# huttered40/capital

Measured on AMD Instinct MI355X. Metric: TFLOP/s (whole node) Cholesky n=65536, algorithmic n^3/3, recursive cholinv factor(), inputs resident in HBM, higher is better.
Workload: dtype f64

## Files before the change

### capital_amd/csrc/gemm_f64.hip

```cpp
#include "capi_internal.h"
#include "gemm_plan.h"
#include <type_traits>

extern "C" int capi_internal_copy2d(capi_handle_t h, int64_t m, int64_t n, const double* A, int64_t lda, double* B, int64_t ldb);

typedef double d4_t __attribute__((ext_vector_type(4)));
typedef double d2_t __attribute__((ext_vector_type(2)));

namespace {

constexpr int NTHREADS = 256;
using gemm_plan::BK, gemm_plan::SK;
template <int TS> struct tile_cfg {
  static constexpr int TILE_LDS = TS * SK;
  static constexpr int STAGE_LDS = 2 * TILE_LDS;
  static constexpr int NQ = TS / 32;
  static constexpr int SUB = TS / 32;
};
constexpr int GROUP_M = 8;
template <int TS> __device__ __forceinline__ int rc_r(int tid, int q) { return 16 * ((tid >> 6) * (TS / 64) + (q >> 1)) + 2 * (tid & 7); }
__device__ __forceinline__ int rc_k(int tid, int q) { return 8 * (q & 1) + ((tid >> 3) & 7); }

struct GemmArgs {
  const double* A;
  const double* B;
  double* C;
  int64_t lda, ldb, ldc;
  int M, N, K;
  double alpha, beta;
  int out_uplo;
  int tri_side;
  int tri_eff_upper;
  int tri_unit;
  int a_vec, b_vec;
  int splitk, k_per_split;
  int k_rotate;
  double* slab;
  int64_t slab_ld, slab_stride;
  int tiles_m, tiles_n, ntiles;
  int batch;
  int64_t sa, sb, sc;
  int tail_base, tail_tm, tail_tn;
  int ts;
  int no_skip;
  int share_ab;
  int tri_dense;
  int tri_koff;
  int tri_block;
  int pid_base;
  int order;
  int a_tiled, c_tiled;
  unsigned long long* stamp;
};

__device__ __forceinline__ void stamp_begin(const GemmArgs& p) {
  if (p.stamp && threadIdx.x == 0) atomicMin(p.stamp, (unsigned long long)wall_clock64());
}
__device__ __forceinline__ void stamp_end(const GemmArgs& p) {
  if (p.stamp && threadIdx.x == 0) atomicMin(p.stamp + 1, ~(unsigned long long)wall_clock64());
}

template <int TS, bool KC>
__device__ __forceinline__ void panel_load(const double* __restrict__ X, int64_t ld, int r0, int R, int k0, int kend,
                                           int tid, bool vec_ok, d2_t (&v)[TS / 32]) {
  constexpr int NQ = TS / 32;
  if (KC) {
    const int kp = tid & 7, rb = tid >> 3;
    const int k = k0 + 2 * kp;
#pragma unroll
    for (int q = 0; q < NQ; ++q) {
      const int r = r0 + rb + 32 * q;
      d2_t val = {0.0, 0.0};
      if (r < R) {
        const double* p = X + (int64_t)r * ld + k;
        if (vec_ok && k + 1 < kend) {
          val = *(const d2_t*)p;
        } else {
          if (k < kend) val.x = p[0];
          if (k + 1 < kend) val.y = p[1];
        }
      }
      v[q] = val;
    }
  } else {
#pragma unroll
    for (int q = 0; q < NQ; ++q) {
      const int r = r0 + rc_r<TS>(tid, q);
      const int k = k0 + rc_k(tid, q);
      d2_t val = {0.0, 0.0};
      if (k < kend) {
        const double* p = X + (int64_t)k * ld + r;
        if (vec_ok && r + 1 < R) {
          val = *(const d2_t*)p;
        } else {
          if (r < R) val.x = p[0];
          if (r + 1 < R) val.y = p[1];
        }
      }
      v[q] = val;
    }
  }
}

template <int TS>
__device__ __forceinline__ void panel_load_fast(const double* __restrict__ base, int64_t s1, int64_t s2, d2_t (&v)[TS / 32]) {
#pragma unroll
  for (int q = 0; q < TS / 32; ++q) v[q] = *(const d2_t*)(base + (q & 1) * s1 + (q >> 1) * s2);
}

template <int TS, bool KC>
__device__ __forceinline__ void panel_mask(int r0, int k0, int tid, bool keep_ge, bool unit, d2_t (&v)[TS / 32]) {
#pragma unroll
  for (int q = 0; q < TS / 32; ++q) {
    int r[2], k[2];
    if (KC) {
      r[0] = r[1] = r0 + (tid >> 3) + 32 * q;
      k[0] = k0 + 2 * (tid & 7);
      k[1] = k[0] + 1;
    } else {
      r[0] = r0 + rc_r<TS>(tid, q);
      r[1] = r[0] + 1;
      k[0] = k[1] = k0 + rc_k(tid, q);
    }
    double e0 = v[q].x, e1 = v[q].y;
    if (keep_ge ? (k[0] < r[0]) : (k[0] > r[0])) e0 = 0.0;
    if (keep_ge ? (k[1] < r[1]) : (k[1] > r[1])) e1 = 0.0;
    if (unit) {
      if (k[0] == r[0]) e0 = 1.0;
      if (k[1] == r[1]) e1 = 1.0;
    }
    v[q].x = e0;
    v[q].y = e1;
  }
}

template <int TS, bool KC>
__device__ __forceinline__ void panel_store(double* __restrict__ L, int tid, const d2_t (&v)[TS / 32]) {
  if (KC) {
    const int kp = tid & 7, rb = tid >> 3;
#pragma unroll
    for (int q = 0; q < TS / 32; ++q) *(d2_t*)&L[(rb + 32 * q) * SK + 2 * kp] = v[q];
  } else {
#pragma unroll
    for (int q = 0; q < TS / 32; ++q) {
      double* d = &L[rc_r<TS>(tid, q) * SK + rc_k(tid, q)];
      d[0] = v[q].x;
      d[SK] = v[q].y;
    }
  }
}

__device__ __forceinline__ d2_t frag_read(const double* __restrict__ L, int row, int u, int g) {
  return *(const d2_t*)&L[row * SK + 8 * u + 2 * g];
}

template <int SUB, int COMP, bool ALL>
__device__ __forceinline__ void mfma_step(d4_t (&acc)[SUB][SUB], const d2_t (&af)[SUB], const d2_t (&bf)[SUB], unsigned keep) {
  constexpr unsigned FULL = (1u << (SUB * SUB)) - 1u;
  if (ALL || keep == FULL) {
#pragma unroll
    for (int a = 0; a < SUB; ++a)
#pragma unroll
      for (int b = 0; b < SUB; ++b)
        acc[a][b] = __builtin_amdgcn_mfma_f64_16x16x4f64(COMP ? bf[b].y : bf[b].x, COMP ? af[a].y : af[a].x, acc[a][b], 0, 0, 0);
  } else {
#pragma unroll
    for (int a = 0; a < SUB; ++a)
#pragma unroll
      for (int b = 0; b < SUB; ++b)
        if (keep & (1u << (a * SUB + b)))
          acc[a][b] = __builtin_amdgcn_mfma_f64_16x16x4f64(COMP ? bf[b].y : bf[b].x, COMP ? af[a].y : af[a].x, acc[a][b], 0, 0, 0);
  }
}

__device__ __forceinline__ void tile_of_dims(int out_uplo, int nm, int nn, int t, int& ti, int& tj, int order = 0) {
  if (out_uplo >= 0 && (order & 1)) {
    int first = 0, gsz = GROUP_M;
    for (;; first += GROUP_M) {
      gsz = min(nn - first, GROUP_M);
      const int cnt = gsz * (gsz + 1) / 2 + gsz * (nn - first - gsz);
      if (t < cnt || first + GROUP_M >= nn) break;
      t -= cnt;
    }
    const int ntri = gsz * (gsz + 1) / 2;
    int lo, hi;
    if (t < ntri) {
      hi = 0;
      while ((hi + 1) * (hi + 2) / 2 <= t) ++hi;
      lo = first + t - hi * (hi + 1) / 2;
      hi += first;
    } else {
      t -= ntri;
      hi = first + gsz + t / gsz;
      lo = first + t % gsz;
    }
    if (out_uplo == CAPI_UPPER) { ti = lo; tj = hi; } else { ti = hi; tj = lo; }
  } else if (out_uplo < 0) {
    const int in_group = GROUP_M * nn;
    const int group = t / in_group;
    const int first_m = group * GROUP_M;
    const int gsz = min(nm - first_m, GROUP_M);
    const int loc = t - group * in_group;
    ti = first_m + loc % gsz;
    tj = loc / gsz;
  } else {
    int hi = (int)((sqrt(8.0 * (double)t + 1.0) - 1.0) * 0.5);
    while ((int64_t)hi * (hi + 1) / 2 > t) --hi;
    while ((int64_t)(hi + 1) * (hi + 2) / 2 <= t) ++hi;
    const int lo = t - (int)((int64_t)hi * (hi + 1) / 2);
    if (out_uplo == CAPI_UPPER) { ti = lo; tj = hi; } else { ti = hi; tj = lo; }
  }
}

__device__ __forceinline__ void tile_of(const GemmArgs& p, int t, int& ti, int& tj) {
  if (p.tail_base > 0) {
    int ti128, tj128;
    tile_of_dims(p.out_uplo, p.tail_tm, p.tail_tn, p.tail_base + (t >> 2), ti128, tj128, p.order);
    ti = 2 * ti128 + (t & 1);
    tj = 2 * tj128 + ((t >> 1) & 1);
  } else {
    tile_of_dims(p.out_uplo, p.tiles_m, p.tiles_n, t, ti, tj, p.order);
  }
}

__device__ __forceinline__ void trmm_tile_of(const GemmArgs& p, int r, int& ti, int& tj) {
  const bool left = p.tri_side == CAPI_LEFT;
  const int nfree = left ? p.tiles_n : p.tiles_m, ntri = left ? p.tiles_m : p.tiles_n;
  int b = r / nfree;
  const int a = r - b * nfree;
  const bool longest_last = left ? !p.tri_eff_upper : (p.tri_eff_upper != 0);
  if (longest_last) b = ntri - 1 - b;
  ti = left ? b : a;
  tj = left ? a : b;
}

template <int TS, bool AK, bool BKC>
__global__ __launch_bounds__(NTHREADS, TS == 128 ? 2 : 4) void dgemm_tile_kernel(const GemmArgs p) {
  constexpr int BM = TS, BN = TS, SUB = tile_cfg<TS>::SUB, NQ = tile_cfg<TS>::NQ;
  constexpr int NW = NQ * ((AK ? 1 : 2) + (BKC ? 1 : 2));
  constexpr int TILE_LDS = tile_cfg<TS>::TILE_LDS, STAGE_LDS = tile_cfg<TS>::STAGE_LDS;
  extern __shared__ __attribute__((aligned(16))) double lds[];
  const int tid = threadIdx.x;
  const int lane = tid & 63, wave = tid >> 6;
  const int r16 = lane & 15, g = lane >> 4;
  const int wm = wave & 1, wn = wave >> 1;
  stamp_begin(p);

  const int nblk = gridDim.x, bid = blockIdx.x;
  const int xcd = bid & 7, qq = nblk >> 3, rr = nblk & 7;
  const int pid = p.pid_base + (xcd < rr ? xcd * (qq + 1) : rr * (qq + 1) + (xcd - rr) * qq) + (bid >> 3);
  int z = pid / p.ntiles;
  int ti, tj;
  if (p.tri_side >= 0 && p.splitk == 1 && !p.tri_block) { z = 0; trmm_tile_of(p, bid, ti, tj); }
  else tile_of(p, pid - z * p.ntiles, ti, tj);
  if (p.tail_base > 0) {
    if (ti >= p.tiles_m || tj >= p.tiles_n) return;
    if (p.out_uplo == CAPI_UPPER && ti > tj) return;
    if (p.out_uplo == CAPI_LOWER && tj > ti) return;
  }
  const int i0 = ti * BM, j0 = tj * BN;

  int klo = 0, khi = p.K;
  if (p.tri_side == CAPI_LEFT) {
    if (p.tri_eff_upper) klo = i0; else khi = min(p.K, i0 + BM);
  } else if (p.tri_side == CAPI_RIGHT) {
    if (p.tri_eff_upper) khi = min(p.K, p.tri_koff + j0 + BN); else klo = j0;
  }
  constexpr int kstep = BK;
  if (p.splitk > 1) {
    klo = max(klo, z * p.k_per_split);
    khi = min(khi, (z + 1) * p.k_per_split);
  }
  const int ntk = khi > klo ? (khi - klo + kstep - 1) / kstep : 0;
  const bool maskA = p.tri_side == CAPI_LEFT && !p.tri_dense, maskB = p.tri_side == CAPI_RIGHT && !p.tri_dense;
  const bool shareB = AK == BKC && p.share_ab && ti == tj;
  const bool keep_ge = (p.tri_side == CAPI_LEFT) == (p.tri_eff_upper != 0);

  d4_t acc[SUB][SUB];
#pragma unroll
  for (int a = 0; a < SUB; ++a)
#pragma unroll
    for (int b = 0; b < SUB; ++b) acc[a][b] = (d4_t){0.0, 0.0, 0.0, 0.0};

  const bool interior = (i0 + BM <= p.M) && (j0 + BN <= p.N) && p.a_vec && p.b_vec;
  const double* fa = AK ? p.A + (int64_t)(i0 + (tid >> 3)) * p.lda + klo + 2 * (tid & 7)
                     : p.A + (int64_t)(klo + rc_k(tid, 0)) * p.lda + i0 + rc_r<TS>(tid, 0);
  const double* fb = BKC ? p.B + (int64_t)(j0 + (tid >> 3)) * p.ldb + klo + 2 * (tid & 7)
                     : p.B + (int64_t)(klo + rc_k(tid, 0)) * p.ldb + j0 + rc_r<TS>(tid, 0);
  const int64_t qsa = AK ? 32 * p.lda : 8 * p.lda;
  const int64_t qsa2 = AK ? 64 * p.lda : 16;
  const int64_t qsb = BKC ? 32 * p.ldb : 8 * p.ldb;
  const int64_t qsb2 = BKC ? 64 * p.ldb : 16;
  const int64_t ksa = AK ? kstep : (int64_t)kstep * p.lda, ksb = BKC ? kstep : (int64_t)kstep * p.ldb;

  unsigned out_keep = (1u << (SUB * SUB)) - 1u;
  if (p.out_uplo >= 0 && ti == tj && !p.no_skip) {
#pragma unroll
    for (int a = 0; a < SUB; ++a)
#pragma unroll
      for (int b = 0; b < SUB; ++b) {
        const int rlo = wm * (TS / 2) + 16 * a, clo = wn * (TS / 2) + 16 * b;
        const bool on = p.out_uplo == CAPI_UPPER ? (rlo <= clo + 15) : (rlo + 15 >= clo);
        if (!on) out_keep &= ~(1u << (a * SUB + b));
      }
  }

  const int rot = (p.k_rotate && p.splitk > 1 && ntk > 1) ? (int)((int64_t)z * ntk / p.splitk) : 0;
  const int kfirst = klo + rot * kstep;
  d2_t ra[NQ], rb[NQ];
  if (ntk > 0) {
    panel_load<TS, AK>(p.A, p.lda, i0, p.M, kfirst, khi, tid, p.a_vec, ra);
    if (!shareB) panel_load<TS, BKC>(p.B, p.ldb, j0, p.N, kfirst, khi, tid, p.b_vec, rb);
    if (maskA && klo < i0 + BM && klo + BK > i0) panel_mask<TS, AK>(i0, klo, tid, keep_ge, p.tri_unit, ra);
    if (maskB && klo < j0 + BN && klo + BK > j0) panel_mask<TS, BKC>(j0, klo, tid, keep_ge, p.tri_unit, rb);
    panel_store<TS, AK>(lds, tid, ra);
    if (!shareB) panel_store<TS, BKC>(lds + TILE_LDS, tid, rb);
  }
  __syncthreads();

  int par = 0;
  auto iterate = [&](const int t, const int tnext, auto fast_tag) {
    constexpr bool FAST = decltype(fast_tag)::value;
    const double* La = lds + par * STAGE_LDS;
    const double* Lb = shareB ? La : La + TILE_LDS;
    const int kn = klo + tnext * kstep;
    const bool more = FAST || (tnext >= 0);
    if (FAST) {
      fa += ksa;
      fb += ksb;
      __builtin_amdgcn_s_setprio(1);
      panel_load_fast<TS>(fa, qsa, qsa2, ra);
      panel_load_fast<TS>(fb, qsb, qsb2, rb);
    } else if (more) {
      panel_load<TS, AK>(p.A, p.lda, i0, p.M, kn, khi, tid, p.a_vec, ra);
      if (!shareB) panel_load<TS, BKC>(p.B, p.ldb, j0, p.N, kn, khi, tid, p.b_vec, rb);
    }
    unsigned keep = (1u << (SUB * SUB)) - 1u;
    if (!FAST) {
      keep = out_keep;
      const int kk = klo + t * kstep;
      const bool band = p.tri_side == CAPI_LEFT ? (kk < i0 + BM && kk + BK > i0) : (kk < j0 + BN && kk + BK > j0);
      if (p.tri_side >= 0 && band && !p.no_skip && !p.tri_dense) {
#pragma unroll
        for (int a = 0; a < SUB; ++a)
#pragma unroll
          for (int b = 0; b < SUB; ++b) {
            bool on;
            if (p.tri_side == CAPI_LEFT) {
              const int rlo = i0 + wm * (TS / 2) + 16 * a;
              on = p.tri_eff_upper ? (kk + BK - 1 >= rlo) : (kk <= rlo + 15);
            } else {
              const int clo = j0 + wn * (TS / 2) + 16 * b;
              on = p.tri_eff_upper ? (kk <= clo + 15) : (kk + BK - 1 >= clo);
            }
            if (!on) keep &= ~(1u << (a * SUB + b));
          }
      }
    }
#pragma unroll
    for (int u = 0; u < 2; ++u) {
      d2_t af[SUB], bf[SUB];
#pragma unroll
      for (int a = 0; a < SUB; ++a) af[a] = frag_read(La, wm * (TS / 2) + a * 16 + r16, u, g);
#pragma unroll
      for (int b = 0; b < SUB; ++b) bf[b] = frag_read(Lb, wn * (TS / 2) + b * 16 + r16, u, g);
      if (!FAST) __builtin_amdgcn_s_setprio(1);
      mfma_step<SUB, 0, FAST>(acc, af, bf, keep);
      mfma_step<SUB, 1, FAST>(acc, af, bf, keep);
      if (FAST && u == 1) {
        double* Na = lds + (par ^ 1) * STAGE_LDS;
        panel_store<TS, AK>(Na, tid, ra);
        panel_store<TS, BKC>(Na + TILE_LDS, tid, rb);
        __builtin_amdgcn_sched_group_barrier(0x100, 2 * SUB, 0);
#pragma unroll
        for (int i = 0; i < 2 * NQ; ++i) {
          __builtin_amdgcn_sched_group_barrier(0x008, (SUB * SUB) / (2 * NQ), 0);
          __builtin_amdgcn_sched_group_barrier(0x020, 1, 0);
        }
#pragma unroll
        for (int i = 0; i < 2 * SUB; ++i) {
          __builtin_amdgcn_sched_group_barrier(0x008, (SUB * SUB) / (2 * SUB), 0);
          __builtin_amdgcn_sched_group_barrier(0x100, 1, 0);
        }
#pragma unroll
        for (int i = 0; i < NW; ++i) {
          __builtin_amdgcn_sched_group_barrier(0x008, (2 * SUB * SUB) / NW > 0 ? (2 * SUB * SUB) / NW : 1, 0);
          __builtin_amdgcn_sched_group_barrier(0x200, 1, 0);
        }
      }
      if (!FAST || u == 1) __builtin_amdgcn_s_setprio(0);
    }
    if (more && !FAST) {
      if (maskA && kn < i0 + BM && kn + BK > i0) panel_mask<TS, AK>(i0, kn, tid, keep_ge, p.tri_unit, ra);
      if (maskB && kn < j0 + BN && kn + BK > j0) panel_mask<TS, BKC>(j0, kn, tid, keep_ge, p.tri_unit, rb);
      double* Na = lds + (par ^ 1) * STAGE_LDS;
      panel_store<TS, AK>(Na, tid, ra);
      if (!shareB) panel_store<TS, BKC>(Na + TILE_LDS, tid, rb);
    }
    par ^= 1;
    __syncthreads();
  };
  const int nfast = (interior && khi - klo >= BK) ? (khi - klo - BK) / kstep : 0;
  int tb0 = ntk, tb1 = ntk;
  if (p.tri_side >= 0 && !p.tri_dense) {
    const int d0 = p.tri_side == CAPI_LEFT ? i0 : j0;
    tb0 = d0 > klo ? (d0 - klo) / BK : 0;
    tb1 = d0 + TS > klo ? (d0 + TS - klo + BK - 1) / BK : 0;
  }
  const double* const fa0 = fa;
  const double* const fb0 = fb;
  for (int seg = 0; seg < 2; ++seg) {
    const int tb = seg == 0 ? rot : 0, te = seg == 0 ? ntk : rot;
    const int after = (seg == 0 && rot > 0) ? 0 : -1;
    fa = fa0 + (int64_t)tb * ksa;
    fb = fb0 + (int64_t)tb * ksb;
    const int lim = min(nfast, te - 1);
    int t = tb;
    while (t < te) {
      const int fe = t + 1 < tb0 ? min(tb0 - 1, lim) : (t >= tb1 ? lim : t);
      for (; t < fe; ++t) iterate(t, t + 1, std::true_type{});
      const int ge = (t < tb1 && tb1 < lim) ? tb1 : te;
      const int t_in = t;
      for (; t < ge; ++t) iterate(t, t + 1 < te ? t + 1 : after, std::false_type{});
      fa += (int64_t)(t - t_in) * ksa;
      fb += (int64_t)(t - t_in) * ksb;
    }
  }

  auto element_ok = [&](int i, int j) {
    bool ok = (i < p.M) && (j < p.N);
    if (p.out_uplo == CAPI_UPPER) ok = ok && (i <= j);
    if (p.out_uplo == CAPI_LOWER) ok = ok && (i >= j);
    return ok;
  };
  if (p.splitk > 1) {
#pragma unroll
    for (int a = 0; a < SUB; ++a) {
      const int i = i0 + wm * (TS / 2) + a * 16 + r16;
#pragma unroll
      for (int b = 0; b < SUB; ++b)
#pragma unroll
        for (int reg = 0; reg < 4; ++reg) {
          const int j = j0 + wn * (TS / 2) + b * 16 + g + 4 * reg;
          if (element_ok(i, j)) p.slab[(int64_t)z * p.slab_stride + i + (int64_t)j * p.slab_ld] = acc[a][b][reg];
        }
    }
  } else if (p.beta == 0.0) {
#pragma unroll
    for (int a = 0; a < SUB; ++a) {
      const int i = i0 + wm * (TS / 2) + a * 16 + r16;
#pragma unroll
      for (int b = 0; b < SUB; ++b)
#pragma unroll
        for (int reg = 0; reg < 4; ++reg) {
          const int j = j0 + wn * (TS / 2) + b * 16 + g + 4 * reg;
          if (element_ok(i, j)) p.C[i + (int64_t)j * p.ldc] = p.alpha * acc[a][b][reg];
        }
    }
  } else {
#pragma unroll
    for (int a = 0; a < SUB; ++a) {
      const int i = i0 + wm * (TS / 2) + a * 16 + r16;
      double old[SUB][4];
#pragma unroll
      for (int b = 0; b < SUB; ++b)
#pragma unroll
        for (int reg = 0; reg < 4; ++reg) {
          const int j = j0 + wn * (TS / 2) + b * 16 + g + 4 * reg;
          const bool ok = element_ok(i, j);
          old[b][reg] = *(ok ? p.C + i + (int64_t)j * p.ldc : p.C);
        }
#pragma unroll
      for (int b = 0; b < SUB; ++b)
#pragma unroll
        for (int reg = 0; reg < 4; ++reg) {
          const int j = j0 + wn * (TS / 2) + b * 16 + g + 4 * reg;
          if (element_ok(i, j)) p.C[i + (int64_t)j * p.ldc] = p.alpha * acc[a][b][reg] + p.beta * old[b][reg];
        }
    }
  }
  stamp_end(p);
}

template <bool AK, bool BKC>
__global__ __launch_bounds__(NTHREADS, 2) void dtrmm_pair_kernel(const GemmArgs p) {
  constexpr int TS = 128, BM = TS, BN = TS, SUB = tile_cfg<TS>::SUB, NQ = tile_cfg<TS>::NQ;
  constexpr int NW = NQ * ((AK ? 1 : 2) + (BKC ? 1 : 2));
  constexpr int TILE_LDS = tile_cfg<TS>::TILE_LDS, STAGE_LDS = tile_cfg<TS>::STAGE_LDS;
  constexpr int kstep = BK;
  extern __shared__ __attribute__((aligned(16))) double lds[];
  const int tid = threadIdx.x;
  const int lane = tid & 63, wave = tid >> 6;
  const int r16 = lane & 15, g = lane >> 4;
  const int wm = wave & 1, wn = wave >> 1;
  stamp_begin(p);

  const int nblk = gridDim.x, bid = blockIdx.x;
  const int xcd = bid & 7, qq = nblk >> 3, rr = nblk & 7;
  const int pid = p.pid_base + (xcd < rr ? xcd * (qq + 1) : rr * (qq + 1) + (xcd - rr) * qq) + (bid >> 3);
  const bool left = p.tri_side == CAPI_LEFT;
  const int ntri = left ? p.tiles_m : p.tiles_n, nfree = left ? p.tiles_n : p.tiles_m, npair = ntri >> 1;
  int pb, fr;
  if (left) tile_of_dims(-1, npair, nfree, pid, pb, fr); else tile_of_dims(-1, nfree, npair, pid, fr, pb);
  const bool anchor0 = left ? !p.tri_eff_upper : (p.tri_eff_upper != 0);
  const bool maskA = left, maskB = !left;
  const bool keep_ge = left == (p.tri_eff_upper != 0);
  const int64_t ksa = AK ? kstep : (int64_t)kstep * p.lda, ksb = BKC ? kstep : (int64_t)kstep * p.ldb;
  const int64_t qsa = AK ? 32 * p.lda : 8 * p.lda;
  const int64_t qsa2 = AK ? 64 * p.lda : 16;
  const int64_t qsb = BKC ? 32 * p.ldb : 8 * p.ldb;
  const int64_t qsb2 = BKC ? 64 * p.ldb : 16;

  for (int ph = 0; ph < 2; ++ph) {
    const bool asc = (ph == 0) == anchor0;
    const int bt = asc ? pb : ntri - 1 - pb;
    const int ti = left ? bt : fr, tj = left ? fr : bt;
    const int i0 = ti * BM, j0 = tj * BN, d0 = left ? i0 : j0;
    const int klo = anchor0 ? 0 : d0, khi = anchor0 ? d0 + TS : p.K;
    const int ntk = (khi - klo) / kstep;
    const int tb0 = (d0 - klo) / BK, tb1 = tb0 + TS / BK;

    d4_t acc[SUB][SUB];
#pragma unroll
    for (int a = 0; a < SUB; ++a)
#pragma unroll
      for (int c = 0; c < SUB; ++c) acc[a][c] = (d4_t){0.0, 0.0, 0.0, 0.0};

    const double* const fa0 = AK ? p.A + (int64_t)(i0 + (tid >> 3)) * p.lda + klo + 2 * (tid & 7)
                              : p.A + (int64_t)(klo + rc_k(tid, 0)) * p.lda + i0 + rc_r<TS>(tid, 0);
    const double* const fb0 = BKC ? p.B + (int64_t)(j0 + (tid >> 3)) * p.ldb + klo + 2 * (tid & 7)
                              : p.B + (int64_t)(klo + rc_k(tid, 0)) * p.ldb + j0 + rc_r<TS>(tid, 0);
    const double* fa = fa0;
    const double* fb = fb0;
    const int64_t sa = asc ? ksa : -ksa, sb = asc ? ksb : -ksb;
    const int dir = asc ? 1 : -1;
    int t = asc ? 0 : ntk - 1;

    d2_t ra[NQ], rb[NQ];
    {
      const int kf = klo + t * kstep;
      panel_load<TS, AK>(p.A, p.lda, i0, p.M, kf, khi, tid, 1, ra);
      panel_load<TS, BKC>(p.B, p.ldb, j0, p.N, kf, khi, tid, 1, rb);
      if (maskA && t >= tb0 && t < tb1) panel_mask<TS, AK>(i0, kf, tid, keep_ge, p.tri_unit, ra);
      if (maskB && t >= tb0 && t < tb1) panel_mask<TS, BKC>(j0, kf, tid, keep_ge, p.tri_unit, rb);
      panel_store<TS, AK>(lds, tid, ra);
      panel_store<TS, BKC>(lds + TILE_LDS, tid, rb);
    }
    __syncthreads();

    int par = 0;
    auto iterate = [&](const int tc, const int tnext, auto fast_tag) {
      constexpr bool FAST = decltype(fast_tag)::value;
      const double* La = lds + par * STAGE_LDS;
      const double* Lb = La + TILE_LDS;
      const int kn = klo + tnext * kstep;
      const bool more = FAST || (tnext >= 0);
      if (FAST) {
        fa += sa;
        fb += sb;
        __builtin_amdgcn_s_setprio(1);
        panel_load_fast<TS>(fa, qsa, qsa2, ra);
        panel_load_fast<TS>(fb, qsb, qsb2, rb);
      } else if (more) {
        panel_load<TS, AK>(p.A, p.lda, i0, p.M, kn, khi, tid, 1, ra);
        panel_load<TS, BKC>(p.B, p.ldb, j0, p.N, kn, khi, tid, 1, rb);
      }
      unsigned keep = (1u << (SUB * SUB)) - 1u;
      if (!FAST) {
        const int kk = klo + tc * kstep;
        if (tc >= tb0 && tc < tb1 && !p.no_skip) {
#pragma unroll
          for (int a = 0; a < SUB; ++a)
#pragma unroll
            for (int c = 0; c < SUB; ++c) {
              bool on;
              if (left) {
                const int rlo = i0 + wm * (TS / 2) + 16 * a;
                on = p.tri_eff_upper ? (kk + BK - 1 >= rlo) : (kk <= rlo + 15);
              } else {
                const int clo = j0 + wn * (TS / 2) + 16 * c;
                on = p.tri_eff_upper ? (kk <= clo + 15) : (kk + BK - 1 >= clo);
              }
              if (!on) keep &= ~(1u << (a * SUB + c));
            }
        }
      }
#pragma unroll
      for (int u = 0; u < 2; ++u) {
        d2_t af[SUB], bf[SUB];
#pragma unroll
        for (int a = 0; a < SUB; ++a) af[a] = frag_read(La, wm * (TS / 2) + a * 16 + r16, u, g);
#pragma unroll
        for (int c = 0; c < SUB; ++c) bf[c] = frag_read(Lb, wn * (TS / 2) + c * 16 + r16, u, g);
        if (!FAST) __builtin_amdgcn_s_setprio(1);
        mfma_step<SUB, 0, FAST>(acc, af, bf, keep);
        mfma_step<SUB, 1, FAST>(acc, af, bf, keep);
        if (FAST && u == 1) {
          double* Na = lds + (par ^ 1) * STAGE_LDS;
          panel_store<TS, AK>(Na, tid, ra);
          panel_store<TS, BKC>(Na + TILE_LDS, tid, rb);
          __builtin_amdgcn_sched_group_barrier(0x100, 2 * SUB, 0);
#pragma unroll
          for (int i = 0; i < 2 * NQ; ++i) {
            __builtin_amdgcn_sched_group_barrier(0x008, (SUB * SUB) / (2 * NQ), 0);
            __builtin_amdgcn_sched_group_barrier(0x020, 1, 0);
          }
#pragma unroll
          for (int i = 0; i < 2 * SUB; ++i) {
            __builtin_amdgcn_sched_group_barrier(0x008, (SUB * SUB) / (2 * SUB), 0);
            __builtin_amdgcn_sched_group_barrier(0x100, 1, 0);
          }
#pragma unroll
          for (int i = 0; i < NW; ++i) {
            __builtin_amdgcn_sched_group_barrier(0x008, (2 * SUB * SUB) / NW > 0 ? (2 * SUB * SUB) / NW : 1, 0);
            __builtin_amdgcn_sched_group_barrier(0x200, 1, 0);
          }
        }
        if (!FAST || u == 1) __builtin_amdgcn_s_setprio(0);
      }
      if (more && !FAST) {
        if (maskA && tnext >= tb0 && tnext < tb1) panel_mask<TS, AK>(i0, kn, tid, keep_ge, p.tri_unit, ra);
        if (maskB && tnext >= tb0 && tnext < tb1) panel_mask<TS, BKC>(j0, kn, tid, keep_ge, p.tri_unit, rb);
        double* Na = lds + (par ^ 1) * STAGE_LDS;
        panel_store<TS, AK>(Na, tid, ra);
        panel_store<TS, BKC>(Na + TILE_LDS, tid, rb);
      }
      par ^= 1;
      __syncthreads();
    };
    auto fast_run = [&](int tc) -> int {
      if (asc) return tc < tb0 ? max(0, min(tb0, ntk) - 1 - tc) : (tc >= tb1 ? max(0, ntk - 1 - tc) : 0);
      return tc >= tb1 ? tc - tb1 : (tc < tb0 ? tc : 0);
    };
    while (t >= 0 && t < ntk) {
      const int nf = fast_run(t);
      fa = fa0 + (int64_t)t * ksa;
      fb = fb0 + (int64_t)t * ksb;
      for (int q = 0; q < nf; ++q, t += dir) iterate(t, t + dir, std::true_type{});
      while (t >= 0 && t < ntk) {
        const int tn = t + dir;
        iterate(t, (tn >= 0 && tn < ntk) ? tn : -1, std::false_type{});
        t = tn;
        if (t >= 0 && t < ntk && fast_run(t) > 0) break;
      }
    }

#pragma unroll
    for (int a = 0; a < SUB; ++a) {
      const int i = i0 + wm * (TS / 2) + a * 16 + r16;
#pragma unroll
      for (int c = 0; c < SUB; ++c)
#pragma unroll
        for (int reg = 0; reg < 4; ++reg) {
          const int j = j0 + wn * (TS / 2) + c * 16 + g + 4 * reg;
          p.C[i + (int64_t)j * p.ldc] = p.alpha * acc[a][c][reg];
        }
    }
  }
  stamp_end(p);
}

__global__ void splitk_reduce_kernel(const double* __restrict__ slab, int64_t slab_ld, int64_t slab_stride, int splitk,
                                     double* __restrict__ C, int64_t ldc, int M, int N, double alpha, double beta, int out_uplo) {
  const int i = blockIdx.x * blockDim.x + threadIdx.x;
  if (i >= M) return;
  for (int j = blockIdx.y; j < N; j += gridDim.y) {
    if (out_uplo == CAPI_UPPER && i > j) continue;
    if (out_uplo == CAPI_LOWER && i < j) continue;
    double s = 0.0;
    for (int z = 0; z < splitk; ++z) s += slab[(int64_t)z * slab_stride + i + (int64_t)j * slab_ld];
    double* c = C + i + (int64_t)j * ldc;
    double r = alpha * s;
    if (beta != 0.0) r += beta * (*c);
    *c = r;
  }
}

__global__ __launch_bounds__(256) void splitk_reduce_wide_kernel(const double* __restrict__ slab, int64_t slab_ld, int64_t slab_stride,
                                                                 int splitk, double* __restrict__ C, int64_t ldc, int M, int N,
                                                                 double alpha, double beta, int out_uplo) {
  __shared__ double part[4][64];
  const int il = threadIdx.x & 63, zl = threadIdx.x >> 6;
  const int i = blockIdx.x * 64 + il, j = blockIdx.y;
  const bool live = i < M && !(out_uplo == CAPI_UPPER && i > j) && !(out_uplo == CAPI_LOWER && i < j);
  double s = 0.0;
  if (live) {
    const double* src = slab + i + (int64_t)j * slab_ld;
    int z = zl;
    for (; z + 28 < splitk; z += 32) {
      double v[8];
#pragma unroll
      for (int q = 0; q < 8; ++q) v[q] = src[(int64_t)(z + 4 * q) * slab_stride];
#pragma unroll
      for (int q = 0; q < 8; ++q) s += v[q];
    }
    for (; z < splitk; z += 4) s += src[(int64_t)z * slab_stride];
  }
  part[zl][il] = s;
  __syncthreads();
  if (zl == 0 && live) {
    const double t = ((part[0][il] + part[1][il]) + part[2][il]) + part[3][il];
    double* c = C + i + (int64_t)j * ldc;
    double r = alpha * t;
    if (beta != 0.0) r += beta * (*c);
    *c = r;
  }
}

__global__ void scale_kernel(double* __restrict__ C, int64_t ldc, int M, int N, double beta, int out_uplo) {
  const int i = blockIdx.x * blockDim.x + threadIdx.x;
  if (i >= M) return;
  for (int j = blockIdx.y; j < N; j += gridDim.y) {
    if (out_uplo == CAPI_UPPER && i > j) continue;
    if (out_uplo == CAPI_LOWER && i < j) continue;
    double* c = C + i + (int64_t)j * ldc;
    *c = beta == 0.0 ? 0.0 : beta * (*c);
  }
}

typedef void (*gemm_kernel_t)(const GemmArgs);

using gemm_plan::ST, gemm_plan::SKC, gemm_plan::SQK, gemm_plan::SLD;

template <bool KC>
__device__ __forceinline__ void small_load(const double* __restrict__ X, int64_t ld, int r0, int R, int kc, int kend, int tid,
                                           bool vec_ok, int quarter, d2_t (&v)[16]) {
#pragma unroll
  for (int qq = 0; qq < 4; ++qq) {
    const int q = 4 * quarter + qq;
    int r[2], k[2];
    if (KC) { r[0] = r[1] = r0 + (tid >> 3); k[0] = kc + 2 * (tid & 7) + 16 * q; k[1] = k[0] + 1; }
    else { r[0] = r0 + 2 * (tid & 15); r[1] = r[0] + 1; k[0] = k[1] = kc + (tid >> 4) + 16 * q; }
    const double* ptr = KC ? X + (int64_t)r[0] * ld + k[0] : X + (int64_t)k[0] * ld + r[0];
    const bool in = r[1] < R && k[1] < kend && vec_ok;
    v[q] = *(const d2_t*)(in ? ptr : X);
  }
}

template <bool KC>
__device__ __forceinline__ void small_load_fast(const double* __restrict__ X, int64_t ld, int r0, int kc, int npieces, int tid,
                                                int quarter, d2_t (&v)[16]) {
  const double* ptr = KC ? X + (int64_t)(r0 + (tid >> 3)) * ld + kc + 2 * (tid & 7) : X + (int64_t)(kc + (tid >> 4)) * ld + r0 + 2 * (tid & 15);
  const int64_t sq = KC ? 16 : 16 * ld;
#pragma unroll
  for (int qq = 0; qq < 4; ++qq) {
    const int q = 4 * quarter + qq;
    v[q] = q < npieces ? *(const d2_t*)(ptr + q * sq) : (d2_t){0.0, 0.0};
  }
}

template <bool KC>
__device__ __forceinline__ void small_fix(const double* __restrict__ X, int64_t ld, int r0, int R, int kc, int kend, int tid,
                                          bool vec_ok, bool tri, bool keep_ge, bool unit, int quarter, d2_t (&v)[16]) {
#pragma unroll
  for (int qq = 0; qq < 4; ++qq) {
    const int q = 4 * quarter + qq;
    int r[2], k[2];
    if (KC) { r[0] = r[1] = r0 + (tid >> 3); k[0] = kc + 2 * (tid & 7) + 16 * q; k[1] = k[0] + 1; }
    else { r[0] = r0 + 2 * (tid & 15); r[1] = r[0] + 1; k[0] = k[1] = kc + (tid >> 4) + 16 * q; }
    const bool in = r[1] < R && k[1] < kend && vec_ok;
    d2_t val = v[q];
    if (!in) {
      const double* ptr = KC ? X + (int64_t)r[0] * ld + k[0] : X + (int64_t)k[0] * ld + r[0];
      val = (d2_t){0.0, 0.0};
      if (r[0] < R && k[0] < kend) val.x = ptr[0];
      if (r[1] < R && k[1] < kend) val.y = ptr[1];
    }
    const int kq = kc + 16 * q;
    if (tri && kq < r0 + ST && kq + 16 > r0) {
      if (keep_ge ? (k[0] < r[0]) : (k[0] > r[0])) val.x = 0.0;
      if (keep_ge ? (k[1] < r[1]) : (k[1] > r[1])) val.y = 0.0;
      if (unit) {
        if (k[0] == r[0]) val.x = 1.0;
        if (k[1] == r[1]) val.y = 1.0;
      }
    }
    v[q] = val;
  }
}

template <bool KC>
__device__ __forceinline__ void small_store(double* __restrict__ L, int tid, int quarter, const d2_t (&v)[16]) {
#pragma unroll
  for (int qq = 0; qq < 4; ++qq) {
    const int q = 4 * quarter + qq;
    if (KC) {
      const int k = 2 * (tid & 7) + 16 * q, r = tid >> 3;
      L[k * SLD + r] = v[q].x;
      L[(k + 1) * SLD + r] = v[q].y;
    } else {
      const int k = (tid >> 4) + 16 * q, r = 2 * (tid & 15);
      *(d2_t*)&L[k * SLD + r] = v[q];
    }
  }
}

// ... 863 lines not shown
```

Before: 55.50.

## Rewrite fast K-loop with buffer loads and interleaved LDS store/MFMA schedule

Replaces the per-iteration fast path in the GEMM and TRMM-pair kernels with a dedicated fast_run loop. The loop issues raw buffer loads through a 32-bit lane offset and interleaves per-piece LDS stores, next-tile global loads and second-half fragment reads among the MFMAs using sched_group_barrier. The goal is to hide global load latency and LDS traffic behind matrix math and to cut 64-bit address arithmetic. It also adds a leading-dimension limit so the 32-bit offsets cannot overflow, and it raises register pressure and scheduling complexity.

```diff
diff --git a/capital_amd/csrc/gemm_f64.hip b/capital_amd/csrc/gemm_f64.hip
--- a/capital_amd/csrc/gemm_f64.hip
+++ b/capital_amd/csrc/gemm_f64.hip
@@ -102,12 +102,6 @@
   }
 }
 
-template <int TS>
-__device__ __forceinline__ void panel_load_fast(const double* __restrict__ base, int64_t s1, int64_t s2, d2_t (&v)[TS / 32]) {
-#pragma unroll
-  for (int q = 0; q < TS / 32; ++q) v[q] = *(const d2_t*)(base + (q & 1) * s1 + (q >> 1) * s2);
-}
-
 template <int TS, bool KC>
 __device__ __forceinline__ void panel_mask(int r0, int k0, int tid, bool keep_ge, bool unit, d2_t (&v)[TS / 32]) {
 #pragma unroll
@@ -135,19 +129,20 @@
 }
 
 template <int TS, bool KC>
+__device__ __forceinline__ void piece_store(double* __restrict__ L, int tid, int q, const d2_t v) {
+  if (KC) {
+    *(d2_t*)&L[((tid >> 3) + 32 * q) * SK + 2 * (tid & 7)] = v;
+  } else {
+    double* d = &L[rc_r<TS>(tid, q) * SK + rc_k(tid, q)];
+    d[0] = v.x;
+    d[SK] = v.y;
+  }
+}
+
+template <int TS, bool KC>
 __device__ __forceinline__ void panel_store(double* __restrict__ L, int tid, const d2_t (&v)[TS / 32]) {
-  if (KC) {
-    const int kp = tid & 7, rb = tid >> 3;
-#pragma unroll
-    for (int q = 0; q < TS / 32; ++q) *(d2_t*)&L[(rb + 32 * q) * SK + 2 * kp] = v[q];
-  } else {
-#pragma unroll
-    for (int q = 0; q < TS / 32; ++q) {
-      double* d = &L[rc_r<TS>(tid, q) * SK + rc_k(tid, q)];
-      d[0] = v[q].x;
-      d[SK] = v[q].y;
-    }
-  }
+#pragma unroll
+  for (int q = 0; q < TS / 32; ++q) piece_store<TS, KC>(L, tid, q, v[q]);
 }
 
 __device__ __forceinline__ d2_t frag_read(const double* __restrict__ L, int row, int u, int g) {
@@ -170,6 +165,161 @@
       for (int b = 0; b < SUB; ++b)
         if (keep & (1u << (a * SUB + b)))
           acc[a][b] = __builtin_amdgcn_mfma_f64_16x16x4f64(COMP ? bf[b].y : bf[b].x, COMP ? af[a].y : af[a].x, acc[a][b], 0, 0, 0);
+  }
+}
+
+struct FastSrc {
+  const double* u;
+  unsigned lane;
+  int64_t step;
+  int64_t s1, s2;
+};
+constexpr int64_t FAST_LD_MAX = (int64_t)1 << 24;
+template <int TS, bool KC> __device__ __forceinline__ FastSrc fast_src(const double* X, int64_t ld, int r0, int k0, int64_t step, int tid) {
+  FastSrc s;
+  s.u = KC ? X + (int64_t)r0 * ld + k0 : X + (int64_t)k0 * ld + r0;
+  s.lane = 8u * (KC ? (unsigned)(tid >> 3) * (unsigned)ld + 2u * (tid & 7) : (unsigned)rc_k(tid, 0) * (unsigned)ld + (unsigned)rc_r<TS>(tid, 0));
+  s.step = step;
+  s.s1 = KC ? 32 * ld : 8 * ld;
+  s.s2 = KC ? 64 * ld : 16;
+  return s;
+}
+__device__ __forceinline__ __amdgpu_buffer_rsrc_t panel_rsrc(const double* u) {
+  return __builtin_amdgcn_make_buffer_rsrc((void*)u, 0, -1, 0x00020000);
+}
+__device__ __forceinline__ d2_t piece_load(const double* panel, const FastSrc& s, int q) {
+  return __builtin_bit_cast(d2_t, __builtin_amdgcn_raw_buffer_load_b128(panel_rsrc(panel + (q & 1) * s.s1 + (q >> 1) * s.s2), s.lane, 0, 0));
+}
+
+template <int TS> struct fast_sched {
+  static constexpr int SUB = TS / 32, NP = 2 * (TS / 32), NM = 4 * SUB * SUB, MQ = NM / NP, RD = (NM / 4) / (2 * SUB);
+  static constexpr int piece_after(int m) { return (m + 1 >= MQ / 2 && (m + 1 - MQ / 2) % MQ == 0) ? (m + 1 - MQ / 2) / MQ : -1; }
+  static constexpr int read_after(int m) { return (m + 1 > NM / 4 && m + 1 <= NM / 2 && (m + 1 - NM / 4) % RD == 0) ? (m + 1 - NM / 4) / RD - 1 : -1; }
+};
+
+template <int TS, bool AK, bool BKC>
+__device__ __forceinline__ void fast_run(d4_t (&acc)[TS / 32][TS / 32], double* __restrict__ lds, int& par, const bool shareB,
+                                         const FastSrc sa, const FastSrc sb, const int run_len, const int tid) {
+  const int nf = __builtin_amdgcn_readfirstlane(run_len);
+  using S = fast_sched<TS>;
+  constexpr int SUB = tile_cfg<TS>::SUB, NQ = tile_cfg<TS>::NQ, NM = S::NM;
+  constexpr int TILE_LDS = tile_cfg<TS>::TILE_LDS, STAGE_LDS = tile_cfg<TS>::STAGE_LDS;
+  constexpr unsigned FULL = (1u << (SUB * SUB)) - 1u;
+  const int lane = tid & 63, wave = tid >> 6;
+  const int r16 = lane & 15, g = lane >> 4;
+  int fo_a = ((wave & 1) * (TS / 2) + r16) * SK + 2 * g, fo_b = ((wave >> 1) * (TS / 2) + r16) * SK + 2 * g;
+  int so_a = AK ? (tid >> 3) * SK + 2 * (tid & 7) : rc_r<TS>(tid, 0) * SK + rc_k(tid, 0);
+  asm("" : "+v"(fo_a), "+v"(fo_b), "+v"(so_a));
+  int so_b = so_a;
+  if (AK != BKC) {
+    so_b = BKC ? (tid >> 3) * SK + 2 * (tid & 7) : rc_r<TS>(tid, 0) * SK + rc_k(tid, 0);
+    asm("" : "+v"(so_b));
+  }
+  auto frag = [](const double* L, int fo, int sub, int u) { return *(const d2_t*)&L[fo + sub * 16 * SK + 8 * u]; };
+  auto put = [](double* L, int so, bool kc, int q, const d2_t v) {
+    if (kc) {
+      *(d2_t*)&L[so + 32 * q * SK] = v;
+    } else {
+      double* d = &L[so + 16 * (q >> 1) * SK + 8 * (q & 1)];
+      d[0] = v.x;
+      d[SK] = v.y;
+    }
+  };
+
+  d2_t ra[NQ], rb[NQ];
+  const double* pa = sa.u + sa.step;
+  const double* pb = sb.u + sb.step;
+
+#pragma unroll
+  for (int q = 0; q < NQ; ++q) ra[q] = piece_load(pa, sa, q);
+#pragma unroll
+  for (int q = 0; q < NQ; ++q) rb[q] = piece_load(pb, sb, q);
+
+  for (int i = nf == 1 ? 0 : 1; i < 1; ++i) {
+    const double* La = lds + par * STAGE_LDS;
+    const double* Lb = shareB ? La : La + TILE_LDS;
+    double* Na = lds + (par ^ 1) * STAGE_LDS;
+    __builtin_amdgcn_s_setprio(1);
+#pragma unroll
+    for (int u = 0; u < 2; ++u) {
+      d2_t af[SUB], bf[SUB];
+#pragma unroll
+      for (int a = 0; a < SUB; ++a) af[a] = frag(La, fo_a, a, u);
+#pragma unroll
+      for (int b = 0; b < SUB; ++b) bf[b] = frag(Lb, fo_b, b, u);
+      mfma_step<SUB, 0, true>(acc, af, bf, FULL);
+      mfma_step<SUB, 1, true>(acc, af, bf, FULL);
+    }
+#pragma unroll
+    for (int q = 0; q < NQ; ++q) put(Na, so_a, AK, q, ra[q]);
+#pragma unroll
+    for (int q = 0; q < NQ; ++q) put(Na + TILE_LDS, so_b, BKC, q, rb[q]);
+    constexpr int NW = NQ * ((AK ? 1 : 2) + (BKC ? 1 : 2));
+    __builtin_amdgcn_sched_group_barrier(0x100, 2 * SUB, 0);
+    __builtin_amdgcn_sched_group_barrier(0x008, SUB * SUB, 0);
+#pragma unroll
+    for (int k = 0; k < 2 * SUB; ++k) {
+      __builtin_amdgcn_sched_group_barrier(0x008, (SUB * SUB) / (2 * SUB), 0);
+      __builtin_amdgcn_sched_group_barrier(0x100, 1, 0);
+    }
+#pragma unroll
+    for (int k = 0; k < NW; ++k) {
+      __builtin_amdgcn_sched_group_barrier(0x008, (2 * SUB * SUB) / NW > 0 ? (2 * SUB * SUB) / NW : 1, 0);
+      __builtin_amdgcn_sched_group_barrier(0x200, 1, 0);
+    }
+    __builtin_amdgcn_s_setprio(0);
+    par ^= 1;
+    __syncthreads();
+  }
+
+  for (int i = nf == 1 ? 1 : 0; i < nf; ++i) {
+    const bool more = i + 1 < nf;
+    pa = more ? pa + sa.step : pa;
+    pb = more ? pb + sb.step : pb;
+    const double* const ca = pa;
+    const double* const cb = pb;
+    const double* La = lds + par * STAGE_LDS;
+    const double* Lb = shareB ? La : La + TILE_LDS;
+    double* Na = lds + (par ^ 1) * STAGE_LDS;
+    __builtin_amdgcn_s_setprio(1);
+    d2_t af[2][SUB], bf[2][SUB];
+#pragma unroll
+    for (int a = 0; a < SUB; ++a) af[0][a] = frag(La, fo_a, a, 0);
+#pragma unroll
+    for (int b = 0; b < SUB; ++b) bf[0][b] = frag(Lb, fo_b, b, 0);
+#pragma unroll
+    for (int m = 0; m < NM; ++m) {
+      const int r = S::read_after(m), j = S::piece_after(m);
+      if (r >= 0 && r < SUB) af[1][r] = frag(La, fo_a, r, 1);
+      if (r >= SUB) bf[1][r - SUB] = frag(Lb, fo_b, r - SUB, 1);
+      if (j >= 0 && j < NQ) {
+        put(Na, so_a, AK, j, ra[j]);
+        ra[j] = piece_load(ca, sa, j);
+      }
+      if (j >= NQ) {
+        put(Na + TILE_LDS, so_b, BKC, j - NQ, rb[j - NQ]);
+        rb[j - NQ] = piece_load(cb, sb, j - NQ);
+      }
+    }
+#pragma unroll
+    for (int u = 0; u < 2; ++u) {
+      mfma_step<SUB, 0, true>(acc, af[u], bf[u], FULL);
+      mfma_step<SUB, 1, true>(acc, af[u], bf[u], FULL);
+    }
+    __builtin_amdgcn_sched_group_barrier(0x100, 2 * SUB, 0);
+#pragma unroll
+    for (int m = 0; m < NM; ++m) {
+      __builtin_amdgcn_sched_group_barrier(0x008, 1, 0);
+      if (S::read_after(m) >= 0) __builtin_amdgcn_sched_group_barrier(0x100, 1, 0);
+      if (S::piece_after(m) >= 0) {
+        if (S::piece_after(m) < NQ) __builtin_amdgcn_sched_group_barrier(0x200, AK ? 1 : 2, 0);
+        else __builtin_amdgcn_sched_group_barrier(0x200, BKC ? 1 : 2, 0);
+        __builtin_amdgcn_sched_group_barrier(0x020, 1, 0);
+      }
+    }
+    __builtin_amdgcn_s_setprio(0);
+    par ^= 1;
+    __syncthreads();
   }
 }
 
@@ -237,7 +387,6 @@
 template <int TS, bool AK, bool BKC>
 __global__ __launch_bounds__(NTHREADS, TS == 128 ? 2 : 4) void dgemm_tile_kernel(const GemmArgs p) {
   constexpr int BM = TS, BN = TS, SUB = tile_cfg<TS>::SUB, NQ = tile_cfg<TS>::NQ;
-  constexpr int NW = NQ * ((AK ? 1 : 2) + (BKC ? 1 : 2));
   constexpr int TILE_LDS = tile_cfg<TS>::TILE_LDS, STAGE_LDS = tile_cfg<TS>::STAGE_LDS;
   extern __shared__ __attribute__((aligned(16))) double lds[];
   const int tid = threadIdx.x;
@@ -282,16 +431,9 @@
 #pragma unroll
     for (int b = 0; b < SUB; ++b) acc[a][b] = (d4_t){0.0, 0.0, 0.0, 0.0};
 
-  const bool interior = (i0 + BM <= p.M) && (j0 + BN <= p.N) && p.a_vec && p.b_vec;
-  const double* fa = AK ? p.A + (int64_t)(i0 + (tid >> 3)) * p.lda + klo + 2 * (tid & 7)
-                     : p.A + (int64_t)(klo + rc_k(tid, 0)) * p.lda + i0 + rc_r<TS>(tid, 0);
-  const double* fb = BKC ? p.B + (int64_t)(j0 + (tid >> 3)) * p.ldb + klo + 2 * (tid & 7)
-                     : p.B + (int64_t)(klo + rc_k(tid, 0)) * p.ldb + j0 + rc_r<TS>(tid, 0);
-  const int64_t qsa = AK ? 32 * p.lda : 8 * p.lda;
-  const int64_t qsa2 = AK ? 64 * p.lda : 16;
-  const int64_t qsb = BKC ? 32 * p.ldb : 8 * p.ldb;
-  const int64_t qsb2 = BKC ? 64 * p.ldb : 16;
+  const bool interior = (i0 + BM <= p.M) && (j0 + BN <= p.N) && p.a_vec && p.b_vec && p.lda < FAST_LD_MAX && p.ldb < FAST_LD_MAX;
   const int64_t ksa = AK ? kstep : (int64_t)kstep * p.lda, ksb = BKC ? kstep : (int64_t)kstep * p.ldb;
+  const FastSrc fa0 = fast_src<TS, AK>(p.A, p.lda, i0, klo, ksa, tid), fb0 = fast_src<TS, BKC>(p.B, p.ldb, j0, klo, ksb, tid);
 
   unsigned out_keep = (1u << (SUB * SUB)) - 1u;
   if (p.out_uplo >= 0 && ti == tj && !p.no_skip) {
@@ -319,43 +461,33 @@
   __syncthreads();
 
   int par = 0;
-  auto iterate = [&](const int t, const int tnext, auto fast_tag) {
-    constexpr bool FAST = decltype(fast_tag)::value;
+  auto iterate = [&](const int t, const int tnext) {
     const double* La = lds + par * STAGE_LDS;
     const double* Lb = shareB ? La : La + TILE_LDS;
     const int kn = klo + tnext * kstep;
-    const bool more = FAST || (tnext >= 0);
-    if (FAST) {
-      fa += ksa;
-      fb += ksb;
-      __builtin_amdgcn_s_setprio(1);
-      panel_load_fast<TS>(fa, qsa, qsa2, ra);
-      panel_load_fast<TS>(fb, qsb, qsb2, rb);
-    } else if (more) {
+    const bool more = tnext >= 0;
+    if (more) {
       panel_load<TS, AK>(p.A, p.lda, i0, p.M, kn, khi, tid, p.a_vec, ra);
       if (!shareB) panel_load<TS, BKC>(p.B, p.ldb, j0, p.N, kn, khi, tid, p.b_vec, rb);
     }
-    unsigned keep = (1u << (SUB * SUB)) - 1u;
-    if (!FAST) {
-      keep = out_keep;
-      const int kk = klo + t * kstep;
-      const bool band = p.tri_side == CAPI_LEFT ? (kk < i0 + BM && kk + BK > i0) : (kk < j0 + BN && kk + BK > j0);
-      if (p.tri_side >= 0 && band && !p.no_skip && !p.tri_dense) {
-#pragma unroll
-        for (int a = 0; a < SUB; ++a)
-#pragma unroll
-          for (int b = 0; b < SUB; ++b) {
-            bool on;
-            if (p.tri_side == CAPI_LEFT) {
-              const int rlo = i0 + wm * (TS / 2) + 16 * a;
-              on = p.tri_eff_upper ? (kk + BK - 1 >= rlo) : (kk <= rlo + 15);
-            } else {
-              const int clo = j0 + wn * (TS / 2) + 16 * b;
-              on = p.tri_eff_upper ? (kk <= clo + 15) : (kk + BK - 1 >= clo);
-            }
-            if (!on) keep &= ~(1u << (a * SUB + b));
+    unsigned keep = out_keep;
+    const int kk = klo + t * kstep;
+    const bool band = p.tri_side == CAPI_LEFT ? (kk < i0 + BM && kk + BK > i0) : (kk < j0 + BN && kk + BK > j0);
+    if (p.tri_side >= 0 && band && !p.no_skip && !p.tri_dense) {
+#pragma unroll
+      for (int a = 0; a < SUB; ++a)
+#pragma unroll
+        for (int b = 0; b < SUB; ++b) {
+          bool on;
+          if (p.tri_side == CAPI_LEFT) {
+            const int rlo = i0 + wm * (TS / 2) + 16 * a;
+            on = p.tri_eff_upper ? (kk + BK - 1 >= rlo) : (kk <= rlo + 15);
+          } else {
+            const int clo = j0 + wn * (TS / 2) + 16 * b;
+            on = p.tri_eff_upper ? (kk <= clo + 15) : (kk + BK - 1 >= clo);
           }
-      }
+          if (!on) keep &= ~(1u << (a * SUB + b));
+        }
     }
 #pragma unroll
     for (int u = 0; u < 2; ++u) {
@@ -364,33 +496,12 @@
       for (int a = 0; a < SUB; ++a) af[a] = frag_read(La, wm * (TS / 2) + a * 16 + r16, u, g);
 #pragma unroll
       for (int b = 0; b < SUB; ++b) bf[b] = frag_read(Lb, wn * (TS / 2) + b * 16 + r16, u, g);
-      if (!FAST) __builtin_amdgcn_s_setprio(1);
-      mfma_step<SUB, 0, FAST>(acc, af, bf, keep);
-      mfma_step<SUB, 1, FAST>(acc, af, bf, keep);
-      if (FAST && u == 1) {
-        double* Na = lds + (par ^ 1) * STAGE_LDS;
-        panel_store<TS, AK>(Na, tid, ra);
-        panel_store<TS, BKC>(Na + TILE_LDS, tid, rb);
-        __builtin_amdgcn_sched_group_barrier(0x100, 2 * SUB, 0);
-#pragma unroll
-        for (int i = 0; i < 2 * NQ; ++i) {
-          __builtin_amdgcn_sched_group_barrier(0x008, (SUB * SUB) / (2 * NQ), 0);
-          __builtin_amdgcn_sched_group_barrier(0x020, 1, 0);
-        }
-#pragma unroll
-        for (int i = 0; i < 2 * SUB; ++i) {
-          __builtin_amdgcn_sched_group_barrier(0x008, (SUB * SUB) / (2 * SUB), 0);
-          __builtin_amdgcn_sched_group_barrier(0x100, 1, 0);
-        }
-#pragma unroll
-        for (int i = 0; i < NW; ++i) {
-          __builtin_amdgcn_sched_group_barrier(0x008, (2 * SUB * SUB) / NW > 0 ? (2 * SUB * SUB) / NW : 1, 0);
-          __builtin_amdgcn_sched_group_barrier(0x200, 1, 0);
-        }
-      }
-      if (!FAST || u == 1) __builtin_amdgcn_s_setprio(0);
-    }
-    if (more && !FAST) {
+      __builtin_amdgcn_s_setprio(1);
+      mfma_step<SUB, 0, false>(acc, af, bf, keep);
+      mfma_step<SUB, 1, false>(acc, af, bf, keep);
+      __builtin_amdgcn_s_setprio(0);
+    }
+    if (more) {
       if (maskA && kn < i0 + BM && kn + BK > i0) panel_mask<TS, AK>(i0, kn, tid, keep_ge, p.tri_unit, ra);
       if (maskB && kn < j0 + BN && kn + BK > j0) panel_mask<TS, BKC>(j0, kn, tid, keep_ge, p.tri_unit, rb);
       double* Na = lds + (par ^ 1) * STAGE_LDS;
@@ -407,23 +518,22 @@
     tb0 = d0 > klo ? (d0 - klo) / BK : 0;
     tb1 = d0 + TS > klo ? (d0 + TS - klo + BK - 1) / BK : 0;
   }
-  const double* const fa0 = fa;
-  const double* const fb0 = fb;
   for (int seg = 0; seg < 2; ++seg) {
     const int tb = seg == 0 ? rot : 0, te = seg == 0 ? ntk : rot;
     const int after = (seg == 0 && rot > 0) ? 0 : -1;
-    fa = fa0 + (int64_t)tb * ksa;
-    fb = fb0 + (int64_t)tb * ksb;
     const int lim = min(nfast, te - 1);
     int t = tb;
     while (t < te) {
       const int fe = t + 1 < tb0 ? min(tb0 - 1, lim) : (t >= tb1 ? lim : t);
-      for (; t < fe; ++t) iterate(t, t + 1, std::true_type{});
+      if (t < fe) {
+        FastSrc fa = fa0, fb = fb0;
+        fa.u += (int64_t)t * ksa;
+        fb.u += (int64_t)t * ksb;
+        fast_run<TS, AK, BKC>(acc, lds, par, shareB, fa, fb, fe - t, tid);
+        t = fe;
+      }
       const int ge = (t < tb1 && tb1 < lim) ? tb1 : te;
-      const int t_in = t;
-      for (; t < ge; ++t) iterate(t, t + 1 < te ? t + 1 : after, std::false_type{});
-      fa += (int64_t)(t - t_in) * ksa;
-      fb += (int64_t)(t - t_in) * ksb;
+      for (; t < ge; ++t) iterate(t, t + 1 < te ? t + 1 : after);
     }
   }
 
@@ -485,7 +595,6 @@
 template <bool AK, bool BKC>
 __global__ __launch_bounds__(NTHREADS, 2) void dtrmm_pair_kernel(const GemmArgs p) {
   constexpr int TS = 128, BM = TS, BN = TS, SUB = tile_cfg<TS>::SUB, NQ = tile_cfg<TS>::NQ;
-  constexpr int NW = NQ * ((AK ? 1 : 2) + (BKC ? 1 : 2));
   constexpr int TILE_LDS = tile_cfg<TS>::TILE_LDS, STAGE_LDS = tile_cfg<TS>::STAGE_LDS;
   constexpr int kstep = BK;
   extern __shared__ __attribute__((aligned(16))) double lds[];
@@ -506,10 +615,7 @@
   const bool maskA = left, maskB = !left;
   const bool keep_ge = left == (p.tri_eff_upper != 0);
   const int64_t ksa = AK ? kstep : (int64_t)kstep * p.lda, ksb = BKC ? kstep : (int64_t)kstep * p.ldb;
-  const int64_t qsa = AK ? 32 * p.lda : 8 * p.lda;
-  const int64_t qsa2 = AK ? 64 * p.lda : 16;
-  const int64_t qsb = BKC ? 32 * p.ldb : 8 * p.ldb;
-  const int64_t qsb2 = BKC ? 64 * p.ldb : 16;
+  const bool fast_ok = p.lda < FAST_LD_MAX && p.ldb < FAST_LD_MAX;
 
   for (int ph = 0; ph < 2; ++ph) {
     const bool asc = (ph == 0) == anchor0;
@@ -526,14 +632,8 @@
 #pragma unroll
       for (int c = 0; c < SUB; ++c) acc[a][c] = (d4_t){0.0, 0.0, 0.0, 0.0};
 
-    const double* const fa0 = AK ? p.A + (int64_t)(i0 + (tid >> 3)) * p.lda + klo + 2 * (tid & 7)
-                              : p.A + (int64_t)(klo + rc_k(tid, 0)) * p.lda + i0 + rc_r<TS>(tid, 0);
-    const double* const fb0 = BKC ? p.B + (int64_t)(j0 + (tid >> 3)) * p.ldb + klo + 2 * (tid & 7)
-                              : p.B + (int64_t)(klo + rc_k(tid, 0)) * p.ldb + j0 + rc_r<TS>(tid, 0);
-    const double* fa = fa0;
-    const double* fb = fb0;
-    const int64_t sa = asc ? ksa : -ksa, sb = asc ? ksb : -ksb;
     const int dir = asc ? 1 : -1;
+    const FastSrc fa0 = fast_src<TS, AK>(p.A, p.lda, i0, klo, dir * ksa, tid), fb0 = fast_src<TS, BKC>(p.B, p.ldb, j0, klo, dir * ksb, tid);
     int t = asc ? 0 : ntk - 1;
 
     d2_t ra[NQ], rb[NQ];
@@ -549,41 +649,32 @@
     __syncthreads();
 
     int par = 0;
-    auto iterate = [&](const int tc, const int tnext, auto fast_tag) {
-      constexpr bool FAST = decltype(fast_tag)::value;
+    auto iterate = [&](const int tc, const int tnext) {
       const double* La = lds + par * STAGE_LDS;
       const double* Lb = La + TILE_LDS;
       const int kn = klo + tnext * kstep;
-      const bool more = FAST || (tnext >= 0);
-      if (FAST) {
-        fa += sa;
-        fb += sb;
-        __builtin_amdgcn_s_setprio(1);
-        panel_load_fast<TS>(fa, qsa, qsa2, ra);
-        panel_load_fast<TS>(fb, qsb, qsb2, rb);
-      } else if (more) {
+      const bool more = tnext >= 0;
+      if (more) {
         panel_load<TS, AK>(p.A, p.lda, i0, p.M, kn, khi, tid, 1, ra);
         panel_load<TS, BKC>(p.B, p.ldb, j0, p.N, kn, khi, tid, 1, rb);
       }
       unsigned keep = (1u << (SUB * SUB)) - 1u;
-      if (!FAST) {
-        const int kk = klo + tc * kstep;
-        if (tc >= tb0 && tc < tb1 && !p.no_skip) {
-#pragma unroll
-          for (int a = 0; a < SUB; ++a)
-#pragma unroll
-            for (int c = 0; c < SUB; ++c) {
-              bool on;
-              if (left) {
-                const int rlo = i0 + wm * (TS / 2) + 16 * a;
-                on = p.tri_eff_upper ? (kk + BK - 1 >= rlo) : (kk <= rlo + 15);
-              } else {
-                const int clo = j0 + wn * (TS / 2) + 16 * c;
-                on = p.tri_eff_upper ? (kk <= clo + 15) : (kk + BK - 1 >= clo);
-              }
-              if (!on) keep &= ~(1u << (a * SUB + c));
+      const int kk = klo + tc * kstep;
+      if (tc >= tb0 && tc < tb1 && !p.no_skip) {
+#pragma unroll
+        for (int a = 0; a < SUB; ++a)
+#pragma unroll
+          for (int c = 0; c < SUB; ++c) {
+            bool on;
+            if (left) {
+              const int rlo = i0 + wm * (TS / 2) + 16 * a;
+              on = p.tri_eff_upper ? (kk + BK - 1 >= rlo) : (kk <= rlo + 15);
+            } else {
+              const int clo = j0 + wn * (TS / 2) + 16 * c;
+              on = p.tri_eff_upper ? (kk <= clo + 15) : (kk + BK - 1 >= clo);
             }
-        }
+            if (!on) keep &= ~(1u << (a * SUB + c));
+          }
       }
 #pragma unroll
       for (int u = 0; u < 2; ++u) {
@@ -592,33 +683,12 @@
         for (int a = 0; a < SUB; ++a) af[a] = frag_read(La, wm * (TS / 2) + a * 16 + r16, u, g);
 #pragma unroll
         for (int c = 0; c < SUB; ++c) bf[c] = frag_read(Lb, wn * (TS / 2) + c * 16 + r16, u, g);
-        if (!FAST) __builtin_amdgcn_s_setprio(1);
-        mfma_step<SUB, 0, FAST>(acc, af, bf, keep);
-        mfma_step<SUB, 1, FAST>(acc, af, bf, keep);
-        if (FAST && u == 1) {
-          double* Na = lds + (par ^ 1) * STAGE_LDS;
-          panel_store<TS, AK>(Na, tid, ra);
-          panel_store<TS, BKC>(Na + TILE_LDS, tid, rb);
-          __builtin_amdgcn_sched_group_barrier(0x100, 2 * SUB, 0);
-#pragma unroll
-          for (int i = 0; i < 2 * NQ; ++i) {
-            __builtin_amdgcn_sched_group_barrier(0x008, (SUB * SUB) / (2 * NQ), 0);
-            __builtin_amdgcn_sched_group_barrier(0x020, 1, 0);
-          }
-#pragma unroll
-          for (int i = 0; i < 2 * SUB; ++i) {
-            __builtin_amdgcn_sched_group_barrier(0x008, (SUB * SUB) / (2 * SUB), 0);
-            __builtin_amdgcn_sched_group_barrier(0x100, 1, 0);
-          }
-#pragma unroll
-          for (int i = 0; i < NW; ++i) {
-            __builtin_amdgcn_sched_group_barrier(0x008, (2 * SUB * SUB) / NW > 0 ? (2 * SUB * SUB) / NW : 1, 0);
-            __builtin_amdgcn_sched_group_barrier(0x200, 1, 0);
-          }
-        }
-        if (!FAST || u == 1) __builtin_amdgcn_s_setprio(0);
-      }
-      if (more && !FAST) {
+        __builtin_amdgcn_s_setprio(1);
+        mfma_step<SUB, 0, false>(acc, af, bf, keep);
+        mfma_step<SUB, 1, false>(acc, af, bf, keep);
+        __builtin_amdgcn_s_setprio(0);
+      }
+      if (more) {
         if (maskA && tnext >= tb0 && tnext < tb1) panel_mask<TS, AK>(i0, kn, tid, keep_ge, p.tri_unit, ra);
         if (maskB && tnext >= tb0 && tnext < tb1) panel_mask<TS, BKC>(j0, kn, tid, keep_ge, p.tri_unit, rb);
         double* Na = lds + (par ^ 1) * STAGE_LDS;
@@ -628,20 +698,25 @@
       par ^= 1;
       __syncthreads();
     };
-    auto fast_run = [&](int tc) -> int {
+    auto fast_len = [&](int tc) -> int {
+      if (!fast_ok) return 0;
       if (asc) return tc < tb0 ? max(0, min(tb0, ntk) - 1 - tc) : (tc >= tb1 ? max(0, ntk - 1 - tc) : 0);
       return tc >= tb1 ? tc - tb1 : (tc < tb0 ? tc : 0);
     };
     while (t >= 0 && t < ntk) {
-      const int nf = fast_run(t);
-      fa = fa0 + (int64_t)t * ksa;
-      fb = fb0 + (int64_t)t * ksb;
-      for (int q = 0; q < nf; ++q, t += dir) iterate(t, t + dir, std::true_type{});
+      const int nf = fast_len(t);
+      if (nf > 0) {
+        FastSrc fa = fa0, fb = fb0;
+        fa.u += (int64_t)t * ksa;
+        fb.u += (int64_t)t * ksb;
+        fast_run<TS, AK, BKC>(acc, lds, par, false, fa, fb, nf, tid);
+        t += dir * nf;
+      }
       while (t >= 0 && t < ntk) {
         const int tn = t + dir;
-        iterate(t, (tn >= 0 && tn < ntk) ? tn : -1, std::false_type{});
+        iterate(t, (tn >= 0 && tn < ntk) ? tn : -1);
         t = tn;
-        if (t >= 0 && t < ntk && fast_run(t) > 0) break;
+        if (t >= 0 && t < ntk && fast_len(t) > 0) break;
       }
     }
 
```

Result: no change. 55.42 (-0.1%).
